# Hansard-T/FHE-Linformer

Measured on AMD Instinct MI355X. Metric: encrypted Linformer-d128 forward ms/sample, lower is better.
Workload: dtype u64

## Files before the change

fhe-linformer_amd/csrc/kernels_ntt.hip:

```cpp
#include <hip/hip_runtime.h>
#include <algorithm>
#include <cstdlib>
#include "kernels.h"

namespace fhelin {

namespace {

struct NttArgs {
    u64* data;
    const u64* src;
    const u64* tw;
    const u64* tw_rows;
    const u64* moduli;
    const u64* ninv;
    const int* limb_tab;
    int tab_len;
    int limb_first;
    int limb_count;
    int log_n;
    int nvec;
    int period;
    int lazy_out;
    int src_group;
    size_t src_group_stride;
    int src_group2;
    size_t src_group2_stride;
    const u64* lift_qlm;
    int lift_limb;
    int vec0;
};

__device__ __forceinline__ size_t src_offset(const NttArgs& a, int vec, int log_n) {
    if (a.src_group > 0) {
        const int g = vec / a.src_group;
        const size_t in = (size_t)(vec % a.src_group) << log_n;
        if (a.src_group2 > 0) return (size_t)(g / a.src_group2) * a.src_group2_stride + (size_t)(g % a.src_group2) * a.src_group_stride + in;
        return (size_t)g * a.src_group_stride + in;
    }
    return (size_t)vec << log_n;
}

constexpr int TILE = 4096;
constexpr int LDS_WORDS = TILE + TILE / 16;

__device__ __forceinline__ int tile_index(int tau, int k, int p) {
    return ((tau >> p) << (p + 4)) | (k << p) | (tau & ((1 << p) - 1));
}
__device__ __forceinline__ int lds_slot(int e) { return e + (e >> 4); }

__device__ __forceinline__ int limb_of(const NttArgs& a, int vec) {
    return a.limb_tab ? a.limb_tab[a.tab_len ? vec % a.tab_len : vec] : a.limb_first + (vec % a.limb_count);
}

typedef u64 u64x2 __attribute__((ext_vector_type(2)));

struct LimbConst {
    u64 q;
    u64 nq;
    u64 q5;
    u32 sh;
    u32 rr;
};

struct RoundTw {
    u64x2 t[15];
};
template <int KB_LO, int KB_HI>
__device__ __forceinline__ void load_round_tw(RoundTw& r, const u64x2* __restrict__ tw, int log_n, int gbase, int hi) {
#pragma unroll
    for (int kb = KB_LO; kb < KB_HI; ++kb) {
        const int m = 1 << (log_n - (gbase + kb) - 1);
        const int tbase = m + (hi << (3 - kb));
#pragma unroll
        for (int j = 0; j < (8 >> kb); ++j) r.t[(8 >> kb) - 1 + j] = tw[tbase + j];
    }
}

__device__ __forceinline__ void load_round_tw_rows(RoundTw& r, const u64x2* __restrict__ trows, int tau) {
#pragma unroll
    for (int s = 0; s < 15; ++s) r.t[s] = trows[s * 256 + tau];
}

template <int KB, bool LAZY>
__device__ __forceinline__ void fwd_stage(u64 (&x)[16], const RoundTw& tw, const LimbConst& c) {
#pragma unroll
    for (int k0 = 0; k0 < 16; ++k0) {
        if (k0 & (1 << KB)) continue;
        const int k1 = k0 | (1 << KB);
        const u64x2 w = tw.t[(8 >> KB) - 1 + (k0 >> (KB + 1))];
        const u64 X = LAZY ? x[k0] : csub_mask(x[k0], c.q5);
#if defined(FHELIN_BFLY15)
        const u64 T = mul_shoup_lazy5(x[k1], w.x, w.y, c.nq);
        x[k0] = X + T;
        x[k1] = X + c.q5 - T;
#else
        const u64 A = mul_shoup_lazy5_add(x[k1], w.x, w.y, c.nq, X);
        x[k0] = A;
        x[k1] = shl1_add(X, c.q5) - A;
#endif
    }
}
template <int KB_LO, int KB_HI, bool LAZY>
__device__ __forceinline__ void fwd_round(u64 (&x)[16], const RoundTw& tw, const LimbConst& c) {
    if constexpr (KB_LO < KB_HI) {
        fwd_stage<KB_HI - 1, LAZY>(x, tw, c);
        fwd_round<KB_LO, KB_HI - 1, LAZY>(x, tw, c);
    }
}

constexpr int lazy_coef(int s, int c0) { return s == 0 ? c0 : 5 << (s - 1); }

template <int KB, bool FINAL, bool LAZY, int S, int C0>
__device__ __forceinline__ void inv_stage(u64 (&x)[16], const RoundTw& tw, const LimbConst& c, const u64* __restrict__ ninv) {
    const u64 B = c.q * (u64)lazy_coef(S, C0);
    if constexpr (FINAL) {
        const u64 ni = ninv[0], nis = ninv[1], wn = ninv[2], wns = ninv[3];
#pragma unroll
        for (int k0 = 0; k0 < 16; ++k0) {
            if (k0 & (1 << KB)) continue;
            const int k1 = k0 | (1 << KB);
            const u64 X = x[k0], Y = x[k1];
            if (LAZY) {
                x[k0] = csub_mask(reduce_lazy_2q(mul_shoup_lazy5(X + Y, ni, nis, c.nq), c.q, c.sh, c.rr), c.q);
                x[k1] = csub_mask(reduce_lazy_2q(mul_shoup_lazy5(X + B - Y, wn, wns, c.nq), c.q, c.sh, c.rr), c.q);
            } else {
                x[k0] = csub_mask(reduce_lazy_2q(mul_shoup_lazy5(X + Y, ni, nis, c.nq), c.q, c.sh, c.rr), c.q);
                x[k1] = csub_mask(reduce_lazy_2q(mul_shoup_lazy5(X + c.q5 - Y, wn, wns, c.nq), c.q, c.sh, c.rr), c.q);
            }
        }
    } else {
#pragma unroll
        for (int k0 = 0; k0 < 16; ++k0) {
            if (k0 & (1 << KB)) continue;
            const int k1 = k0 | (1 << KB);
            const u64x2 w = tw.t[(8 >> KB) - 1 + (k0 >> (KB + 1))];
            const u64 X = x[k0], Y = x[k1];
            if (LAZY) {
                x[k0] = X + Y;
                x[k1] = mul_shoup_lazy5(X + B - Y, w.x, w.y, c.nq);
            } else {
                x[k0] = csub_mask(X + Y, c.q5);
                x[k1] = mul_shoup_lazy5(X + c.q5 - Y, w.x, w.y, c.nq);
            }
        }
    }
}
template <int KB_LO, int KB_HI, bool LAST, bool LAZY, int S0 = 0, int C0 = 1>
__device__ __forceinline__ void inv_round(u64 (&x)[16], const RoundTw& tw, const LimbConst& c, const u64* __restrict__ ninv) {
    if constexpr (KB_LO < KB_HI) {
        inv_stage<KB_LO, (LAST && KB_LO == KB_HI - 1), LAZY, S0, C0>(x, tw, c, ninv);
        inv_round<KB_LO + 1, KB_HI, LAST, LAZY, S0 + 1, C0>(x, tw, c, ninv);
    }
}

__device__ __forceinline__ void exchange(u64 (&x)[16], u64* lds, int tau, int p_from, int p_to, bool sync_first) {
    if (sync_first) __syncthreads();
#pragma unroll
    for (int k = 0; k < 16; ++k) lds[lds_slot(tile_index(tau, k, p_from))] = x[k];
    __syncthreads();
#pragma unroll
    for (int k = 0; k < 16; ++k) x[k] = lds[lds_slot(tile_index(tau, k, p_to))];
}

__device__ __forceinline__ LimbConst limb_const(const NttArgs& a, int limb) {
    LimbConst c;
    c.q = a.moduli[limb];
    c.nq = 0 - c.q;
    c.q5 = 5 * c.q;
    c.sh = (u32)a.ninv[8 * limb + 4];
    c.rr = (u32)a.ninv[8 * limb + 5];
    return c;
}
#if defined(FHELIN_NTT_FORCE_PATH)
template <bool INVERSE> __device__ __forceinline__ bool lazy_prime(u64) { return FHELIN_NTT_FORCE_PATH; }
#else
template <bool INVERSE> __device__ __forceinline__ bool lazy_prime(u64 q) { return q < (1ull << (INVERSE ? 53 : 57)); }
#endif

template <int A, bool INVERSE, bool LAZY, bool LIFT>
__device__ __forceinline__ void cols_body(const NttArgs& a, u64* lds, int vec, int tile, int limb, const LimbConst& c) {
    constexpr int LOGCW = 12 - A;
    constexpr int CW = 1 << LOGCW;
    constexpr int LOGN = A + 8;
    constexpr int NFULL = A / 4;
    constexpr int REM = A % 4;
    const u64x2* tw = reinterpret_cast<const u64x2*>(a.tw) + ((size_t)limb << LOGN);
    u64* base = a.data + ((size_t)vec << LOGN) + tile * CW;
    const u64* sbase = (LIFT ? a.src + ((size_t)(vec / a.limb_count) << LOGN) : a.src + src_offset(a, vec, LOGN)) + tile * CW;
    const int tau = threadIdx.x;
    u64 x[16];

    auto goff = [](int e) { return ((e >> LOGCW) << 8) | (e & (CW - 1)); };

    if (!INVERSE) {
        constexpr int P0 = LOGCW + A - 4;
#pragma unroll
        for (int k = 0; k < 16; ++k) x[k] = sbase[goff(tile_index(tau, k, P0))];
        if constexpr (LIFT) {
            const u64 half = a.moduli[a.lift_limb] >> 1, qlm = a.lift_qlm[limb];
#pragma unroll
            for (int k = 0; k < 16; ++k) {
                const u64 r = csub_mask(x[k], c.q);
                x[k] = x[k] > half ? sub_mod(r, qlm, c.q) : r;
            }
        }
        RoundTw rt, rn;
        load_round_tw<0, 4>(rt, tw, LOGN, 8 + P0 - LOGCW, tau >> P0);
        fwd_round<0, 4, LAZY>(x, rt, c);
        int p_prev = P0;
        if constexpr (NFULL >= 2) {
            constexpr int P1 = LOGCW + A - 8;
            load_round_tw<0, 4>(rn, tw, LOGN, 8 + P1 - LOGCW, tau >> P1);
            exchange(x, lds, tau, p_prev, P1, false);
            fwd_round<0, 4, LAZY>(x, rn, c);
            p_prev = P1;
        }
        if constexpr (REM > 0) {
            constexpr int PR = LOGCW;
            load_round_tw<0, REM>(rt, tw, LOGN, 8, tau >> PR);
            exchange(x, lds, tau, p_prev, PR, NFULL >= 2);
            fwd_round<0, REM, LAZY>(x, rt, c);
            p_prev = PR;
        }
        constexpr int PL = REM > 0 ? LOGCW : (NFULL >= 2 ? LOGCW + A - 8 : P0);
        (void)p_prev;
#pragma unroll
        for (int k = 0; k < 16; ++k) base[goff(tile_index(tau, k, PL))] = x[k];
    } else {
        const u64* ninv = a.ninv + 8 * limb;
        constexpr int P0 = LOGCW;
#pragma unroll
        for (int k = 0; k < 16; ++k) x[k] = sbase[goff(tile_index(tau, k, P0))];
        RoundTw rt, rn;
        load_round_tw<0, 4>(rt, tw, LOGN, 8, tau >> P0);
        inv_round<0, 4, (NFULL == 1 && REM == 0), LAZY, 0, 2>(x, rt, c, ninv);
        int p_prev = P0;
        if constexpr (NFULL >= 2) {
            constexpr int P1 = LOGCW + 4;
            load_round_tw<0, 4>(rn, tw, LOGN, 8 + 4, tau >> P1);
            exchange(x, lds, tau, p_prev, P1, false);
            inv_round<0, 4, (REM == 0), LAZY, 4, 2>(x, rn, c, ninv);
            p_prev = P1;
        }
        if constexpr (REM > 0) {
            constexpr int PR = 8;
            load_round_tw<4 - REM, 4>(rt, tw, LOGN, 8 + PR - LOGCW, tau >> PR);
            exchange(x, lds, tau, p_prev, PR, NFULL >= 2);
            inv_round<4 - REM, 4, true, LAZY, 4 * NFULL, 2>(x, rt, c, ninv);
            p_prev = PR;
        }
        constexpr int PL = REM > 0 ? 8 : (NFULL >= 2 ? LOGCW + 4 : P0);
        (void)p_prev;
#pragma unroll
        for (int k = 0; k < 16; ++k) base[goff(tile_index(tau, k, PL))] = x[k];
    }
}

template <int A, bool INVERSE, bool LIFT = false>
__global__ __launch_bounds__(256) __attribute__((amdgpu_waves_per_eu(LIFT ? 3 : 4))) void ntt_cols_kernel(NttArgs a) {
    constexpr int LOGTILES = A - 4;
    __shared__ u64 lds[LDS_WORDS];
    const int vec = a.vec0 + (blockIdx.x >> LOGTILES);
    const int tile = blockIdx.x & ((1 << LOGTILES) - 1);
    const int limb = limb_of(a, vec);
    if (limb < 0) return;
    const LimbConst c = limb_const(a, limb);
    if (lazy_prime<INVERSE>(c.q))
        cols_body<A, INVERSE, true, LIFT>(a, lds, vec, tile, limb, c);
    else
        cols_body<A, INVERSE, false, LIFT>(a, lds, vec, tile, limb, c);
}

template <bool INVERSE, bool LAZY, bool EPI>
__device__ __forceinline__ void rows_body(const NttArgs& a, u64* lds, int vec, int tile, int limb, const LimbConst& c,
                                          const NttEpilogue* ep) {
    const int log_n = a.log_n;
    const u64x2* tw = reinterpret_cast<const u64x2*>(a.tw) + ((size_t)limb << log_n);
    const u64x2* trows = reinterpret_cast<const u64x2*>(a.tw_rows) + (((size_t)limb << (log_n - 12)) + tile) * (15 * 256);
    u64* base = a.data + ((size_t)vec << log_n) + ((size_t)tile << 12);
    const u64* sbase = a.src + src_offset(a, vec, log_n) + ((size_t)tile << 12);
    const int tau = threadIdx.x;
    u64 x[16];

    if (!INVERSE) {
#pragma unroll
        for (int k = 0; k < 16; ++k) x[k] = sbase[tile_index(tau, k, 4)];
        RoundTw rt, rn;
        load_round_tw<0, 4>(rt, tw, log_n, 4, (tile << 4) | (tau >> 4));
        fwd_round<0, 4, LAZY>(x, rt, c);
        load_round_tw_rows(rn, trows, tau);
        exchange(x, lds, tau, 4, 0, false);
        fwd_round<0, 4, LAZY>(x, rn, c);
        [[maybe_unused]] u64 av[16];
        [[maybe_unused]] int ell = 0, t = 0, poly = 0;
        if constexpr (EPI) {
            ell = ep->ell;
            t = vec % ell;
            poly = vec / ell;
            const u64* acc = ep->acc + (size_t)poly * ep->acc_poly_stride + ((size_t)t << log_n) + ((size_t)tile << 12);
#pragma unroll
            for (int k = 0; k < 16; ++k) av[k] = acc[tile_index(tau, k, 8)];
        }
        if constexpr (EPI) {
#pragma unroll
            for (int k = 0; k < 16; ++k) x[k] = reduce_lazy_2q(x[k], c.q, c.sh, c.rr);
        } else if (!(LAZY && a.lazy_out && c.q < (1ull << 53))) {
#pragma unroll
            for (int k = 0; k < 16; ++k)
                x[k] = csub_mask(reduce_lazy_2q(x[k], c.q, c.sh, c.rr), c.q);
        }
#if defined(FHELIN_ROWS_DIRECT_STORE)
        if constexpr (!EPI) {
#pragma unroll
            for (int k = 0; k < 16; k += 2) {
                u64x2 v;
                v.x = x[k];
                v.y = x[k + 1];
                reinterpret_cast<u64x2*>(base + 16 * tau)[k >> 1] = v;
            }
            return;
        }
#endif
        exchange(x, lds, tau, 0, 8, true);
        if constexpr (EPI) {
            const int bi = poly >> 1, comp = poly & 1;
            const size_t n = (size_t)1 << log_n;
            const u64 w = ep->w[2 * t], ws = ep->w[2 * t + 1];
            const u64 q2 = 2 * c.q;
#pragma unroll
            for (int k = 0; k < 16; ++k) x[k] = mul_shoup(av[k] + q2 - x[k], w, ws, c.q);
            const u64* add = comp == 0 ? ep->add0 : ep->add1;
            if (add) {
                add += (size_t)bi * ep->add_stride + (size_t)t * n + ((size_t)tile << 12);
#pragma unroll
                for (int k = 0; k < 16; ++k) x[k] = add_mod(x[k], add[tile_index(tau, k, 8)], c.q);
            }
            const size_t row_off = (size_t)(comp * ell + t) * n;
            const u64* post = ep->post ? ep->post + (size_t)bi * ep->post_stride + row_off : nullptr;
            u64* out = ep->out + (size_t)bi * ep->out_stride + row_off;
            const u32* im = ep->per_row ? ep->invmap_row[bi] : ep->invmap;
            if (im) {
#pragma unroll
                for (int k = 0; k < 16; ++k) {
                    const size_t j = im[((size_t)tile << 12) + tile_index(tau, k, 8)];
                    u64 r = x[k];
                    if (post) r = add_mod(r, post[j], c.q);
                    out[j] = r;
                }
            } else {
                out += (size_t)tile << 12;
                if (post) {
                    post += (size_t)tile << 12;
#pragma unroll
                    for (int k = 0; k < 16; ++k) x[k] = add_mod(x[k], post[tile_index(tau, k, 8)], c.q);
                }
#pragma unroll
                for (int k = 0; k < 16; ++k) out[tile_index(tau, k, 8)] = x[k];
            }
        } else {
#pragma unroll
            for (int k = 0; k < 16; ++k) base[tile_index(tau, k, 8)] = x[k];
        }
    } else {
#pragma unroll
        for (int k = 0; k < 16; ++k) x[k] = sbase[tile_index(tau, k, 8)];
        RoundTw rt, rn;
        load_round_tw_rows(rt, trows, tau);
        exchange(x, lds, tau, 8, 0, false);
        inv_round<0, 4, false, LAZY, 0, 1>(x, rt, c, nullptr);
        load_round_tw<0, 4>(rn, tw, log_n, 4, (tile << 4) | (tau >> 4));
        exchange(x, lds, tau, 0, 4, true);
        inv_round<0, 4, false, LAZY, 4, 1>(x, rn, c, nullptr);
        if (LAZY) {
#pragma unroll
            for (int k = 0; k < 16; ++k) x[k] = reduce_lazy_2q(x[k], c.q, c.sh, c.rr);
        }
#pragma unroll
        for (int k = 0; k < 16; ++k) base[tile_index(tau, k, 4)] = x[k];
    }
}

template <bool INVERSE, bool EPI = false>
__global__ __launch_bounds__(256) __attribute__((amdgpu_waves_per_eu(4))) void ntt_rows_kernel(NttArgs a, NttEpilogue ep) {
    __shared__ u64 lds[LDS_WORDS];
    const int logtiles = a.log_n - 12;
    int lid = blockIdx.x;
    const int nblk = gridDim.x;
    if ((nblk & 7) == 0) lid = (lid & 7) * (nblk >> 3) + (lid >> 3);
    int vec, tile;
    if (a.period > 0) {
        const int nper = a.nvec / a.period;
        const int rep = lid % nper, r = lid / nper;
        tile = r & ((1 << logtiles) - 1);
        vec = a.vec0 + rep * a.period + (r >> logtiles);
    } else {
        vec = a.vec0 + (lid >> logtiles);
        tile = lid & ((1 << logtiles) - 1);
    }
    const int limb = limb_of(a, vec);
    if (limb < 0) return;
    const LimbConst c = limb_const(a, limb);
    if (lazy_prime<INVERSE>(c.q))
        rows_body<INVERSE, true, EPI>(a, lds, vec, tile, limb, c, &ep);
    else
        rows_body<INVERSE, false, EPI>(a, lds, vec, tile, limb, c, &ep);
}

template <int A>
void launch_cols(const NttArgs& a, bool inverse, int blocks, hipStream_t s) {
    if (inverse)
        hipLaunchKernelGGL((ntt_cols_kernel<A, true>), dim3(blocks), dim3(256), 0, s, a);
    else if (a.lift_qlm)
        hipLaunchKernelGGL((ntt_cols_kernel<A, false, true>), dim3(blocks), dim3(256), 0, s, a);
    else
        hipLaunchKernelGGL((ntt_cols_kernel<A, false>), dim3(blocks), dim3(256), 0, s, a);
}

}

static void launch_ntt_impl(const DeviceTables& t, const LimbBatch& b, bool inverse, const NttEpilogue* ep, hipStream_t s);

void launch_ntt(const DeviceTables& t, const LimbBatch& b, bool inverse, hipStream_t s) { launch_ntt_impl(t, b, inverse, nullptr, s); }
void launch_ntt_epilogue(const DeviceTables& t, const LimbBatch& b, const NttEpilogue& ep, hipStream_t s) {
    launch_ntt_impl(t, b, false, &ep, s);
}

static void launch_ntt_impl(const DeviceTables& t, const LimbBatch& b, bool inverse, const NttEpilogue* ep, hipStream_t s) {
    if (b.nvec <= 0) return;
    NttArgs a;
    a.data = b.data;
    a.src = b.src ? b.src : b.data;
    a.src_group = b.src ? b.src_group : 0;
    a.src_group_stride = b.src_group_stride;
    a.src_group2 = (b.src && b.src_group > 0) ? b.src_group2 : 0;
    a.src_group2_stride = b.src_group2_stride;
    a.lazy_out = (!inverse && b.lazy_out) ? 1 : 0;
    a.lift_qlm = (!inverse && b.src && b.lift_limb >= 0) ? b.lift_qlm : nullptr;
    a.lift_limb = b.lift_limb;
    a.tw = inverse ? t.tw_inv : t.tw_fwd;
    a.tw_rows = inverse ? t.tw_rows_inv : t.tw_rows_fwd;
    a.moduli = t.moduli;
    a.ninv = t.ninv;
    a.limb_tab = b.limb_tab;
    a.tab_len = b.tab_len;
    a.limb_first = b.limb_first;
    a.limb_count = b.limb_count > 0 ? b.limb_count : 1;
    a.log_n = t.log_n;
    a.nvec = b.nvec;
    const int per = b.limb_tab ? b.tab_len : a.limb_count;
    a.period = (per > 0 && per < b.nvec && b.nvec % per == 0) ? per : 0;
    const int A = t.log_n - 8;
    a.vec0 = 0;
    static const int chunk_mb = [] {
        const char* e = std::getenv("FHELIN_NTT_CHUNK_MB");
        return e ? std::atoi(e) : 0;
    }();
    int chunk = b.nvec;
    if (chunk_mb > 0 && !ep) {
        const size_t vec_bytes = (size_t)8 << t.log_n;
        const int want = (int)std::max<size_t>(1, ((size_t)chunk_mb << 20) / vec_bytes);
        if (b.nvec > want + want / 2) {
            const int per = a.period > 0 ? a.period : 1;
            chunk = std::max(per, want / per * per);
        }
    }
    const int nvec_all = b.nvec, period_all = a.period;
    const u64* src_all = a.src;
    const int sg = a.src_group, sg2 = a.src_group2;
    for (int v0 = 0; v0 < nvec_all; v0 += chunk) {
        a.vec0 = v0;
        a.nvec = std::min(chunk, nvec_all - v0);
        a.period = (period_all > 0 && a.nvec % period_all == 0 && a.nvec > period_all) ? period_all : 0;
        a.src = src_all;
        a.src_group = sg;
        a.src_group2 = sg2;
        const int blocks = a.nvec << (t.log_n - 12);
        auto cols = [&]() {
            switch (A) {
                case 4: launch_cols<4>(a, inverse, blocks, s); break;
                case 5: launch_cols<5>(a, inverse, blocks, s); break;
                case 6: launch_cols<6>(a, inverse, blocks, s); break;
                case 7: launch_cols<7>(a, inverse, blocks, s); break;
                case 8: launch_cols<8>(a, inverse, blocks, s); break;
                case 9: launch_cols<9>(a, inverse, blocks, s); break;
                default: break;
            }
        };
        if (!inverse) {
            cols();
            a.src = a.data;
            a.src_group = 0;
            a.src_group2 = 0;
            if (ep)
                hipLaunchKernelGGL((ntt_rows_kernel<false, true>), dim3(blocks), dim3(256), 0, s, a, *ep);
            else
                hipLaunchKernelGGL((ntt_rows_kernel<false, false>), dim3(blocks), dim3(256), 0, s, a, NttEpilogue());
        } else {
            hipLaunchKernelGGL((ntt_rows_kernel<true, false>), dim3(blocks), dim3(256), 0, s, a, NttEpilogue());
            a.src = a.data;
            a.src_group = 0;
            a.src_group2 = 0;
            cols();
        }
    }
}

}
```

Measured before the change: 227.8.

## Use buffer resource loads/stores with scalar offsets in NTT kernels and relax epilogue reduction

Global loads and stores in the NTT row and column kernels now go through AMD buffer resource descriptors. The constant part of each address is placed in the scalar offset and the per-lane part in the vector offset, which cuts per-element 64-bit VGPR address arithmetic. Block-uniform values such as vec, tile, limb and poly are forced to scalars with readfirstlane. The fused epilogue also skips the lazy reduction by subtracting from a larger multiple of q before the Shoup multiply. This relies on the operands staying within bounds and on a 32-bit buffer offset range, which could overflow for large tensors.

```diff
diff --git a/fhe-linformer_amd/csrc/kernels_ntt.hip b/fhe-linformer_amd/csrc/kernels_ntt.hip
--- a/fhe-linformer_amd/csrc/kernels_ntt.hip
+++ b/fhe-linformer_amd/csrc/kernels_ntt.hip
@@ -44,16 +44,50 @@
 constexpr int TILE = 4096;
 constexpr int LDS_WORDS = TILE + TILE / 16;
 
-__device__ __forceinline__ int tile_index(int tau, int k, int p) {
+__device__ __forceinline__ constexpr int tile_index(int tau, int k, int p) {
     return ((tau >> p) << (p + 4)) | (k << p) | (tau & ((1 << p) - 1));
 }
-__device__ __forceinline__ int lds_slot(int e) { return e + (e >> 4); }
+__device__ __forceinline__ constexpr int lds_slot(int e) { return e + (e >> 4); }
 
 __device__ __forceinline__ int limb_of(const NttArgs& a, int vec) {
     return a.limb_tab ? a.limb_tab[a.tab_len ? vec % a.tab_len : vec] : a.limb_first + (vec % a.limb_count);
 }
 
 typedef u64 u64x2 __attribute__((ext_vector_type(2)));
+
+__device__ __forceinline__ int uniform(int v) { return __builtin_amdgcn_readfirstlane(v); }
+typedef u32 u32x2 __attribute__((ext_vector_type(2)));
+typedef u32 u32x4 __attribute__((ext_vector_type(4)));
+struct Stream {
+    __amdgpu_buffer_rsrc_t r;
+};
+__device__ __forceinline__ Stream stream(const void* ubase) {
+    const u64 v = reinterpret_cast<u64>(ubase);
+    const u32 lo = __builtin_amdgcn_readfirstlane((u32)v), hi = __builtin_amdgcn_readfirstlane((u32)(v >> 32));
+    Stream s;
+    s.r = __builtin_amdgcn_make_buffer_rsrc(reinterpret_cast<void*>(((u64)hi << 32) | lo), 0, 0xffffffff, 0x00020000);
+    return s;
+}
+__device__ __forceinline__ u32 ld32(const Stream& s, u32 lane, int K, int soff = 0) {
+    return __builtin_amdgcn_raw_buffer_load_b32(s.r, lane + (K & 4095), soff + (K & ~4095), 0);
+}
+__device__ __forceinline__ u64 ld64(const Stream& s, u32 lane, int K, int soff = 0) {
+    const u32x2 v = __builtin_amdgcn_raw_buffer_load_b64(s.r, lane + (K & 4095), soff + (K & ~4095), 0);
+    return ((u64)v.y << 32) | v.x;
+}
+__device__ __forceinline__ u64x2 ld128(const Stream& s, u32 lane, int K, int soff = 0) {
+    const u32x4 v = __builtin_amdgcn_raw_buffer_load_b128(s.r, lane + (K & 4095), soff + (K & ~4095), 0);
+    u64x2 r;
+    r.x = ((u64)v.y << 32) | v.x;
+    r.y = ((u64)v.w << 32) | v.z;
+    return r;
+}
+__device__ __forceinline__ void st64(const Stream& s, u32 lane, int K, u64 x, int soff = 0) {
+    u32x2 v;
+    v.x = (u32)x;
+    v.y = (u32)(x >> 32);
+    __builtin_amdgcn_raw_buffer_store_b64(v, s.r, lane + (K & 4095), soff + (K & ~4095), 0);
+}
 
 struct LimbConst {
     u64 q;
@@ -67,19 +101,21 @@
     u64x2 t[15];
 };
 template <int KB_LO, int KB_HI>
-__device__ __forceinline__ void load_round_tw(RoundTw& r, const u64x2* __restrict__ tw, int log_n, int gbase, int hi) {
+__device__ __forceinline__ void load_round_tw(RoundTw& r, const Stream& tw, int log_n, int gbase, int hi_u, u32 hi_lane) {
 #pragma unroll
     for (int kb = KB_LO; kb < KB_HI; ++kb) {
         const int m = 1 << (log_n - (gbase + kb) - 1);
-        const int tbase = m + (hi << (3 - kb));
-#pragma unroll
-        for (int j = 0; j < (8 >> kb); ++j) r.t[(8 >> kb) - 1 + j] = tw[tbase + j];
-    }
-}
-
-__device__ __forceinline__ void load_round_tw_rows(RoundTw& r, const u64x2* __restrict__ trows, int tau) {
-#pragma unroll
-    for (int s = 0; s < 15; ++s) r.t[s] = trows[s * 256 + tau];
+        const int soff = 16 * (m + (hi_u << (3 - kb)));
+        const u32 lane = hi_lane << (7 - kb);
+#pragma unroll
+        for (int j = 0; j < (8 >> kb); ++j) r.t[(8 >> kb) - 1 + j] = ld128(tw, lane, 16 * j, soff);
+    }
+}
+
+__device__ __forceinline__ void load_round_tw_rows(RoundTw& r, const Stream& trows, int tau) {
+    const u32 lane = 16u * (u32)tau;
+#pragma unroll
+    for (int s = 0; s < 15; ++s) r.t[s] = ld128(trows, lane, 4096 * s);
 }
 
 template <int KB, bool LAZY>
@@ -156,11 +192,13 @@
 
 __device__ __forceinline__ void exchange(u64 (&x)[16], u64* lds, int tau, int p_from, int p_to, bool sync_first) {
     if (sync_first) __syncthreads();
-#pragma unroll
-    for (int k = 0; k < 16; ++k) lds[lds_slot(tile_index(tau, k, p_from))] = x[k];
+    u64* const from = lds + lds_slot(tile_index(tau, 0, p_from));
+#pragma unroll
+    for (int k = 0; k < 16; ++k) from[lds_slot(tile_index(0, k, p_from))] = x[k];
     __syncthreads();
-#pragma unroll
-    for (int k = 0; k < 16; ++k) x[k] = lds[lds_slot(tile_index(tau, k, p_to))];
+    const u64* const to = lds + lds_slot(tile_index(tau, 0, p_to));
+#pragma unroll
+    for (int k = 0; k < 16; ++k) x[k] = to[lds_slot(tile_index(0, k, p_to))];
 }
 
 __device__ __forceinline__ LimbConst limb_const(const NttArgs& a, int limb) {
@@ -185,18 +223,19 @@
     constexpr int LOGN = A + 8;
     constexpr int NFULL = A / 4;
     constexpr int REM = A % 4;
-    const u64x2* tw = reinterpret_cast<const u64x2*>(a.tw) + ((size_t)limb << LOGN);
-    u64* base = a.data + ((size_t)vec << LOGN) + tile * CW;
-    const u64* sbase = (LIFT ? a.src + ((size_t)(vec / a.limb_count) << LOGN) : a.src + src_offset(a, vec, LOGN)) + tile * CW;
+    const Stream tw = stream(reinterpret_cast<const u64x2*>(a.tw) + ((size_t)limb << LOGN));
+    const Stream base = stream(a.data + ((size_t)vec << LOGN) + tile * CW);
+    const Stream sbase = stream((LIFT ? a.src + ((size_t)(vec / a.limb_count) << LOGN) : a.src + src_offset(a, vec, LOGN)) + tile * CW);
     const int tau = threadIdx.x;
     u64 x[16];
 
-    auto goff = [](int e) { return ((e >> LOGCW) << 8) | (e & (CW - 1)); };
+    auto goff = [](int e) constexpr { return 8 * (((e >> LOGCW) << 8) | (e & (CW - 1))); };
 
     if (!INVERSE) {
         constexpr int P0 = LOGCW + A - 4;
-#pragma unroll
-        for (int k = 0; k < 16; ++k) x[k] = sbase[goff(tile_index(tau, k, P0))];
+        const u32 lane_in = goff(tile_index(tau, 0, P0));
+#pragma unroll
+        for (int k = 0; k < 16; ++k) x[k] = ld64(sbase, lane_in, goff(tile_index(0, k, P0)));
         if constexpr (LIFT) {
             const u64 half = a.moduli[a.lift_limb] >> 1, qlm = a.lift_qlm[limb];
 #pragma unroll
@@ -206,54 +245,57 @@
             }
         }
         RoundTw rt, rn;
-        load_round_tw<0, 4>(rt, tw, LOGN, 8 + P0 - LOGCW, tau >> P0);
+        load_round_tw<0, 4>(rt, tw, LOGN, 8 + P0 - LOGCW, 0, tau >> P0);
         fwd_round<0, 4, LAZY>(x, rt, c);
         int p_prev = P0;
         if constexpr (NFULL >= 2) {
             constexpr int P1 = LOGCW + A - 8;
-            load_round_tw<0, 4>(rn, tw, LOGN, 8 + P1 - LOGCW, tau >> P1);
+            load_round_tw<0, 4>(rn, tw, LOGN, 8 + P1 - LOGCW, 0, tau >> P1);
             exchange(x, lds, tau, p_prev, P1, false);
             fwd_round<0, 4, LAZY>(x, rn, c);
             p_prev = P1;
         }
         if constexpr (REM > 0) {
             constexpr int PR = LOGCW;
-            load_round_tw<0, REM>(rt, tw, LOGN, 8, tau >> PR);
+            load_round_tw<0, REM>(rt, tw, LOGN, 8, 0, tau >> PR);
             exchange(x, lds, tau, p_prev, PR, NFULL >= 2);
             fwd_round<0, REM, LAZY>(x, rt, c);
             p_prev = PR;
         }
         constexpr int PL = REM > 0 ? LOGCW : (NFULL >= 2 ? LOGCW + A - 8 : P0);
         (void)p_prev;
-#pragma unroll
-        for (int k = 0; k < 16; ++k) base[goff(tile_index(tau, k, PL))] = x[k];
+        const u32 lane_out = goff(tile_index(tau, 0, PL));
+#pragma unroll
+        for (int k = 0; k < 16; ++k) st64(base, lane_out, goff(tile_index(0, k, PL)), x[k]);
     } else {
         const u64* ninv = a.ninv + 8 * limb;
         constexpr int P0 = LOGCW;
-#pragma unroll
-        for (int k = 0; k < 16; ++k) x[k] = sbase[goff(tile_index(tau, k, P0))];
+        const u32 lane_in = goff(tile_index(tau, 0, P0));
+#pragma unroll
+        for (int k = 0; k < 16; ++k) x[k] = ld64(sbase, lane_in, goff(tile_index(0, k, P0)));
         RoundTw rt, rn;
-        load_round_tw<0, 4>(rt, tw, LOGN, 8, tau >> P0);
+        load_round_tw<0, 4>(rt, tw, LOGN, 8, 0, tau >> P0);
         inv_round<0, 4, (NFULL == 1 && REM == 0), LAZY, 0, 2>(x, rt, c, ninv);
         int p_prev = P0;
         if constexpr (NFULL >= 2) {
             constexpr int P1 = LOGCW + 4;
-            load_round_tw<0, 4>(rn, tw, LOGN, 8 + 4, tau >> P1);
+            load_round_tw<0, 4>(rn, tw, LOGN, 8 + 4, 0, tau >> P1);
             exchange(x, lds, tau, p_prev, P1, false);
             inv_round<0, 4, (REM == 0), LAZY, 4, 2>(x, rn, c, ninv);
             p_prev = P1;
         }
         if constexpr (REM > 0) {
             constexpr int PR = 8;
-            load_round_tw<4 - REM, 4>(rt, tw, LOGN, 8 + PR - LOGCW, tau >> PR);
+            load_round_tw<4 - REM, 4>(rt, tw, LOGN, 8 + PR - LOGCW, 0, tau >> PR);
             exchange(x, lds, tau, p_prev, PR, NFULL >= 2);
             inv_round<4 - REM, 4, true, LAZY, 4 * NFULL, 2>(x, rt, c, ninv);
             p_prev = PR;
         }
         constexpr int PL = REM > 0 ? 8 : (NFULL >= 2 ? LOGCW + 4 : P0);
         (void)p_prev;
-#pragma unroll
-        for (int k = 0; k < 16; ++k) base[goff(tile_index(tau, k, PL))] = x[k];
+        const u32 lane_out = goff(tile_index(tau, 0, PL));
+#pragma unroll
+        for (int k = 0; k < 16; ++k) st64(base, lane_out, goff(tile_index(0, k, PL)), x[k]);
     }
 }
 
@@ -263,7 +305,7 @@
     __shared__ u64 lds[LDS_WORDS];
     const int vec = a.vec0 + (blockIdx.x >> LOGTILES);
     const int tile = blockIdx.x & ((1 << LOGTILES) - 1);
-    const int limb = limb_of(a, vec);
+    const int limb = uniform(limb_of(a, vec));
     if (limb < 0) return;
     const LimbConst c = limb_const(a, limb);
     if (lazy_prime<INVERSE>(c.q))
@@ -276,18 +318,21 @@
 __device__ __forceinline__ void rows_body(const NttArgs& a, u64* lds, int vec, int tile, int limb, const LimbConst& c,
                                           const NttEpilogue* ep) {
     const int log_n = a.log_n;
-    const u64x2* tw = reinterpret_cast<const u64x2*>(a.tw) + ((size_t)limb << log_n);
-    const u64x2* trows = reinterpret_cast<const u64x2*>(a.tw_rows) + (((size_t)limb << (log_n - 12)) + tile) * (15 * 256);
-    u64* base = a.data + ((size_t)vec << log_n) + ((size_t)tile << 12);
-    const u64* sbase = a.src + src_offset(a, vec, log_n) + ((size_t)tile << 12);
+    const Stream tw = stream(reinterpret_cast<const u64x2*>(a.tw) + ((size_t)limb << log_n));
+    const Stream trows = stream(reinterpret_cast<const u64x2*>(a.tw_rows) + (((size_t)limb << (log_n - 12)) + tile) * (15 * 256));
+    [[maybe_unused]] u64* const vbase = a.data + ((size_t)vec << log_n) + ((size_t)tile << 12);
+    const Stream base = stream(vbase);
+    const Stream sbase = stream(a.src + src_offset(a, vec, log_n) + ((size_t)tile << 12));
     const int tau = threadIdx.x;
+    const u32 lane4 = 8u * (u32)tile_index(tau, 0, 4), lane8 = 8u * (u32)tile_index(tau, 0, 8);
+    auto koff = [](int k, int p) constexpr { return 8 * tile_index(0, k, p); };
     u64 x[16];
 
     if (!INVERSE) {
 #pragma unroll
-        for (int k = 0; k < 16; ++k) x[k] = sbase[tile_index(tau, k, 4)];
+        for (int k = 0; k < 16; ++k) x[k] = ld64(sbase, lane4, koff(k, 4));
         RoundTw rt, rn;
-        load_round_tw<0, 4>(rt, tw, log_n, 4, (tile << 4) | (tau >> 4));
+        load_round_tw<0, 4>(rt, tw, log_n, 4, tile << 4, tau >> 4);
         fwd_round<0, 4, LAZY>(x, rt, c);
         load_round_tw_rows(rn, trows, tau);
         exchange(x, lds, tau, 4, 0, false);
@@ -296,15 +341,23 @@
         [[maybe_unused]] int ell = 0, t = 0, poly = 0;
         if constexpr (EPI) {
             ell = ep->ell;
-            t = vec % ell;
-            poly = vec / ell;
-            const u64* acc = ep->acc + (size_t)poly * ep->acc_poly_stride + ((size_t)t << log_n) + ((size_t)tile << 12);
-#pragma unroll
-            for (int k = 0; k < 16; ++k) av[k] = acc[tile_index(tau, k, 8)];
-        }
+            poly = uniform(vec / ell);
+            t = vec - poly * ell;
+            const Stream acc = stream(ep->acc + (size_t)poly * ep->acc_poly_stride + ((size_t)t << log_n) + ((size_t)tile << 12));
+#pragma unroll
+            for (int k = 0; k < 16; ++k) av[k] = ld64(acc, lane8, koff(k, 8));
+        }
+        [[maybe_unused]] u64 epi_b = 0;
         if constexpr (EPI) {
-#pragma unroll
-            for (int k = 0; k < 16; ++k) x[k] = reduce_lazy_2q(x[k], c.q, c.sh, c.rr);
+            if (LAZY) {
+                epi_b = 86 * c.q;
+            } else if (c.q < (1ull << 60)) {
+                epi_b = 10 * c.q;
+            } else {
+                epi_b = 2 * c.q;
+#pragma unroll
+                for (int k = 0; k < 16; ++k) x[k] = reduce_lazy_2q(x[k], c.q, c.sh, c.rr);
+            }
         } else if (!(LAZY && a.lazy_out && c.q < (1ull << 53))) {
 #pragma unroll
             for (int k = 0; k < 16; ++k)
@@ -317,7 +370,7 @@
                 u64x2 v;
                 v.x = x[k];
                 v.y = x[k + 1];
-                reinterpret_cast<u64x2*>(base + 16 * tau)[k >> 1] = v;
+                reinterpret_cast<u64x2*>(vbase + 16 * tau)[k >> 1] = v;
             }
             return;
         }
@@ -327,49 +380,49 @@
             const int bi = poly >> 1, comp = poly & 1;
             const size_t n = (size_t)1 << log_n;
             const u64 w = ep->w[2 * t], ws = ep->w[2 * t + 1];
-            const u64 q2 = 2 * c.q;
-#pragma unroll
-            for (int k = 0; k < 16; ++k) x[k] = mul_shoup(av[k] + q2 - x[k], w, ws, c.q);
+#pragma unroll
+            for (int k = 0; k < 16; ++k) x[k] = mul_shoup(av[k] + epi_b - x[k], w, ws, c.q);
             const u64* add = comp == 0 ? ep->add0 : ep->add1;
             if (add) {
-                add += (size_t)bi * ep->add_stride + (size_t)t * n + ((size_t)tile << 12);
-#pragma unroll
-                for (int k = 0; k < 16; ++k) x[k] = add_mod(x[k], add[tile_index(tau, k, 8)], c.q);
+                const Stream adds = stream(add + (size_t)bi * ep->add_stride + (size_t)t * n + ((size_t)tile << 12));
+#pragma unroll
+                for (int k = 0; k < 16; ++k) x[k] = add_mod(x[k], ld64(adds, lane8, koff(k, 8)), c.q);
             }
             const size_t row_off = (size_t)(comp * ell + t) * n;
-            const u64* post = ep->post ? ep->post + (size_t)bi * ep->post_stride + row_off : nullptr;
-            u64* out = ep->out + (size_t)bi * ep->out_stride + row_off;
+            const bool has_post = ep->post != nullptr;
+            const Stream post = stream(ep->post + (has_post ? (size_t)bi * ep->post_stride + row_off : 0));
+            const Stream out = stream(ep->out + (size_t)bi * ep->out_stride + row_off);
+            const int toff = tile << 15;
             const u32* im = ep->per_row ? ep->invmap_row[bi] : ep->invmap;
             if (im) {
+                const Stream ims = stream(im + ((size_t)tile << 12));
 #pragma unroll
                 for (int k = 0; k < 16; ++k) {
-                    const size_t j = im[((size_t)tile << 12) + tile_index(tau, k, 8)];
+                    const u32 j8 = 8u * ld32(ims, 4u * (u32)tau, 4 * tile_index(0, k, 8));
                     u64 r = x[k];
-                    if (post) r = add_mod(r, post[j], c.q);
-                    out[j] = r;
+                    if (has_post) r = add_mod(r, ld64(post, j8, 0), c.q);
+                    st64(out, j8, 0, r);
                 }
             } else {
-                out += (size_t)tile << 12;
-                if (post) {
-                    post += (size_t)tile << 12;
-#pragma unroll
-                    for (int k = 0; k < 16; ++k) x[k] = add_mod(x[k], post[tile_index(tau, k, 8)], c.q);
+                if (has_post) {
+#pragma unroll
+                    for (int k = 0; k < 16; ++k) x[k] = add_mod(x[k], ld64(post, lane8, koff(k, 8), toff), c.q);
                 }
 #pragma unroll
-                for (int k = 0; k < 16; ++k) out[tile_index(tau, k, 8)] = x[k];
+                for (int k = 0; k < 16; ++k) st64(out, lane8, koff(k, 8), x[k], toff);
             }
         } else {
 #pragma unroll
-            for (int k = 0; k < 16; ++k) base[tile_index(tau, k, 8)] = x[k];
+            for (int k = 0; k < 16; ++k) st64(base, lane8, koff(k, 8), x[k]);
         }
     } else {
 #pragma unroll
-        for (int k = 0; k < 16; ++k) x[k] = sbase[tile_index(tau, k, 8)];
+        for (int k = 0; k < 16; ++k) x[k] = ld64(sbase, lane8, koff(k, 8));
         RoundTw rt, rn;
         load_round_tw_rows(rt, trows, tau);
         exchange(x, lds, tau, 8, 0, false);
         inv_round<0, 4, false, LAZY, 0, 1>(x, rt, c, nullptr);
-        load_round_tw<0, 4>(rn, tw, log_n, 4, (tile << 4) | (tau >> 4));
+        load_round_tw<0, 4>(rn, tw, log_n, 4, tile << 4, tau >> 4);
         exchange(x, lds, tau, 0, 4, true);
         inv_round<0, 4, false, LAZY, 4, 1>(x, rn, c, nullptr);
         if (LAZY) {
@@ -377,7 +430,7 @@
             for (int k = 0; k < 16; ++k) x[k] = reduce_lazy_2q(x[k], c.q, c.sh, c.rr);
         }
 #pragma unroll
-        for (int k = 0; k < 16; ++k) base[tile_index(tau, k, 4)] = x[k];
+        for (int k = 0; k < 16; ++k) st64(base, lane4, koff(k, 4), x[k]);
     }
 }
 
@@ -398,7 +451,9 @@
         vec = a.vec0 + (lid >> logtiles);
         tile = lid & ((1 << logtiles) - 1);
     }
-    const int limb = limb_of(a, vec);
+    vec = uniform(vec);
+    tile = uniform(tile);
+    const int limb = uniform(limb_of(a, vec));
     if (limb < 0) return;
     const LimbConst c = limb_const(a, limb);
     if (lazy_prime<INVERSE>(c.q))
```

Result: faster. 224.1, median of 6 (-1.6%).
